# Dimitrinov74/Domain-Specific-Image-Compression

Hardware: AMD Instinct MI355X
Metric: 256x256 satellite patches encoded/s per GPU; bpp + MS-SSIM vs reference (higher is better)
Workload: dtype f32 (Winograd contractions as split-bf16 MFMA with fp32 accumulate); 1 GPU; batch=64/GPU 256x256x3 synthetic patches, modelv2 encode->decode (g_a,h_a,round,h_s,Student-t/Gaussian rate,g_s) + bpp + MS-SSIM[.3,.5,.2] on GPU + CDF tables and range coder (z,y strings) on GPU [BASELINE config 3]; global_batch=64, parallelism=per-image sharding x1, one all-reduce of 4 fp64, weights=synthetic seed 1 (checkpoints absent from the reference)

## Files before the change

### domain-specific-image-compression_amd/csrc/conv_first.hip

```cpp
#include <stdlib.h>

#include <type_traits>

#include "common.h"

namespace dsic {

typedef float floatx16 __attribute__((ext_vector_type(16)));
typedef float floatx4 __attribute__((ext_vector_type(4)));
typedef float floatx8 __attribute__((ext_vector_type(8)));
typedef __bf16 bf16x8 __attribute__((ext_vector_type(8)));

__device__ __forceinline__ void first_split8(const floatx8 v, bf16x8& hi, bf16x8& mid) {
  hi = __builtin_convertvector(v, bf16x8);
  const floatx8 back = __builtin_convertvector(hi, floatx8);
  mid = __builtin_convertvector(v - back, bf16x8);
}

template <int C, bool U8 = false, bool BF16 = false>
__global__ __launch_bounds__(256, 2) void conv_first_kernel(
    const void* __restrict__ xv, const float* __restrict__ w, const float* __restrict__ bias,
    const float* __restrict__ beta, const float* __restrict__ gamma, float* __restrict__ out, int B,
    int H, int W, int Cout, int act, int tiles_x, int tiles_y, int layout) {
  const int s2d = layout & 1, cm = layout & DSIC_LAYOUT_CM16;
  constexpr int K = 9 * C;
  constexpr int KP = (K + 1) / 2 * 2;
  constexpr int NS = KP / 2;
  constexpr int TW = 16, TH = 8, WW = TW + 2, WH = TH + 2, RS = 20;
  constexpr int EPI_STRIDE = 36;
  constexpr int WIN_FLOATS = C * WH * RS;
  constexpr int EPI_FLOATS = 4 * 32 * EPI_STRIDE;
  __shared__ __attribute__((aligned(16))) float lds[WIN_FLOATS > EPI_FLOATS ? WIN_FLOATS : EPI_FLOATS];
  constexpr int KB = (K + 15) / 16 * 16;
  constexpr int NKS = KB / 16;
  constexpr int PXB = 4 * KB + 16;
  __shared__ __attribute__((aligned(16))) unsigned char im2col[BF16 ? 128 * PXB : 16];

  const int tid = threadIdx.x, lane = tid & 63;
  const int wave = __builtin_amdgcn_readfirstlane(tid >> 6);
  const int h = lane >> 5, l31 = lane & 31;
  int bx = blockIdx.x;
  const int tile_x = bx % tiles_x;
  bx /= tiles_x;
  const int tile_y = bx % tiles_y;
  const int n = bx / tiles_y;
  const int ox0 = tile_x * TW, oy0 = tile_y * TH;

  const int col = wave * 32 + l31;
  const bool colok = col < Cout;
  float b[BF16 ? 1 : NS];
  int aoff[BF16 ? 1 : NS];
  int abase[4];
  bf16x8 bhi[BF16 ? NKS : 1], bmid[BF16 ? NKS : 1];
  if (BF16) {
#pragma unroll
    for (int ks = 0; ks < NKS; ++ks) {
      floatx8 wv;
#pragma unroll
      for (int j = 0; j < 8; ++j) {
        const int k = ks * 16 + h * 8 + j;
        wv[j] = (colok && k < K) ? w[(size_t)col * K + k] : 0.f;
      }
      first_split8(wv, bhi[ks], bmid[ks]);
    }
  } else {
#pragma unroll
    for (int s = 0; s < NS; ++s) {
      const int k = 2 * s + h;
      b[s] = (colok && k < K) ? w[(size_t)col * K + k] : 0.f;
    }
#pragma unroll
    for (int s = 0; s < NS; ++s) {
      int k = 2 * s + h;
      if (k >= K) k = 0;
      const int c = k / 9, t = k % 9;
      aoff[s] = (c * WH + t / 3) * RS + t % 3;
    }
#pragma unroll
    for (int m = 0; m < 4; ++m) {
      const int r = m * 32 + l31;
      abase[m] = (r / TW) * RS + r % TW;
    }
  }

  if (U8) {
    const unsigned char* xin = (const unsigned char*)xv + (size_t)n * C * H * W;
    for (int i = tid; i < C * WH * WW; i += 256) {
      const int c = i % C, xx = (i / C) % WW, r = i / (C * WW);
      const int gy = oy0 - 1 + r, gx = ox0 - 1 + xx;
      float v = 0.f;
      if (gy >= 0 && gy < H && gx >= 0 && gx < W) v = (float)xin[((size_t)gy * W + gx) * C + c] / 255.0f;
      lds[(c * WH + r) * RS + xx] = v;
    }
  } else {
    const float* xin = (const float*)xv + (size_t)n * C * H * W;
    for (int i = tid; i < C * WH * WW; i += 256) {
      const int c = i / (WH * WW), r = (i / WW) % WH, xx = i % WW;
      const int gy = oy0 - 1 + r, gx = ox0 - 1 + xx;
      float v = 0.f;
      if (gy >= 0 && gy < H && gx >= 0 && gx < W) v = xin[((size_t)c * H + gy) * W + gx];
      lds[(c * WH + r) * RS + xx] = v;
    }
  }
  __syncthreads();

  floatx16 acc[4];
#pragma unroll
  for (int m = 0; m < 4; ++m)
#pragma unroll
    for (int e = 0; e < 16; ++e) acc[m][e] = 0.f;
  if (BF16) {
    const int px = tid & 127, half = tid >> 7;
    const int pbase = (px / TW) * RS + px % TW;
    auto build = [&](auto half_tag) {
      constexpr int HALF = decltype(half_tag)::value;
#pragma unroll
      for (int oo = 0; oo < NKS; ++oo) {
        const int o = 2 * oo + HALF;
        floatx8 v;
#pragma unroll
        for (int j = 0; j < 8; ++j) {
          const int k = 8 * o + j;
          const int c = k / 9, t = k % 9;
          v[j] = k < K ? lds[pbase + (c * WH + t / 3) * RS + t % 3] : 0.f;
        }
        bf16x8 vh, vm;
        first_split8(v, vh, vm);
        *(bf16x8*)(im2col + px * PXB + o * 16) = vh;
        *(bf16x8*)(im2col + px * PXB + 2 * KB + o * 16) = vm;
      }
    };
    if (half == 0)
      build(std::integral_constant<int, 0>{});
    else
      build(std::integral_constant<int, 1>{});
    __syncthreads();
#pragma unroll
    for (int m = 0; m < 4; ++m) {
      const unsigned char* ap = im2col + (m * 32 + l31) * PXB + h * 16;
#pragma unroll
      for (int ks = 0; ks < NKS; ++ks) {
        const bf16x8 ah = *(const bf16x8*)(ap + ks * 32);
        const bf16x8 am = *(const bf16x8*)(ap + 2 * KB + ks * 32);
        acc[m] = __builtin_amdgcn_mfma_f32_32x32x16_bf16(ah, bmid[ks], acc[m], 0, 0, 0);
        acc[m] = __builtin_amdgcn_mfma_f32_32x32x16_bf16(am, bhi[ks], acc[m], 0, 0, 0);
        acc[m] = __builtin_amdgcn_mfma_f32_32x32x16_bf16(ah, bhi[ks], acc[m], 0, 0, 0);
      }
    }
  } else {
#pragma unroll
    for (int s = 0; s < NS; ++s) {
      float a[4];
#pragma unroll
      for (int m = 0; m < 4; ++m) a[m] = lds[abase[m] + aoff[s]];
#pragma unroll
      for (int m = 0; m < 4; ++m) acc[m] = __builtin_amdgcn_mfma_f32_32x32x2f32(a[m], b[s], acc[m], 0, 0, 0);
    }
  }
  __syncthreads();

  const float bs = colok ? bias[col] : 0.f;
  float be = 1.f, ga = 0.f;
  if (colok && act == DSIC_ACT_GDN) {
    be = beta[col];
    ga = gamma[col];
  }
  float* epi = lds + wave * (32 * EPI_STRIDE);
#pragma unroll
  for (int m = 0; m < 4; ++m) {
#pragma unroll
    for (int e = 0; e < 16; e += 2) {
      dsic_float2 v = {acc[m][e], acc[m][e + 1]};
      v = v + dsic_float2{bs, bs};
      if (act == DSIC_ACT_GDN) {
        v = gdn_pair<false>(v, dsic_float2{be, be}, dsic_float2{ga, ga});
      } else if (act == DSIC_ACT_RELU) {
        v[0] = v[0] > 0.f ? v[0] : 0.f;
        v[1] = v[1] > 0.f ? v[1] : 0.f;
      }
#pragma unroll
      for (int k = 0; k < 2; ++k) {
        const int rr = ((e + k) & 3) + 8 * ((e + k) >> 2) + 4 * h;
        epi[rr * EPI_STRIDE + l31] = v[k];
      }
    }
    __builtin_amdgcn_s_waitcnt(0xc07f);
    __builtin_amdgcn_wave_barrier();
    const int c4 = (lane & 7) * 4;
    const int nn = wave * 32 + c4;
#pragma unroll
    for (int i = 0; i < 4; ++i) {
      const int rr = (lane >> 3) + 8 * i;
      const floatx4 v = *(const floatx4*)(epi + rr * EPI_STRIDE + c4);
      const int r = m * 32 + rr;
      const int ox = ox0 + r % TW, oy = oy0 + r / TW;
      if (oy < H && ox < W && nn < Cout) {
        const int64_t pix = s2d ? (int64_t)(oy >> 1) * (W >> 1) + (ox >> 1) : (int64_t)oy * W + ox;
        const int64_t npix = s2d ? (int64_t)(H >> 1) * (W >> 1) : (int64_t)H * W;
        const int Co = s2d ? 4 * Cout : Cout, ch = s2d ? ((oy & 1) * 2 + (ox & 1)) * Cout + nn : nn;
        const size_t o = cm ? (size_t)(((int64_t)n * Co + (ch & ~15)) * npix + pix * 16 + (ch & 15))
                            : (size_t)(((int64_t)n * npix + pix) * Co + ch);
        __builtin_nontemporal_store(v, (floatx4*)(out + o));
      }
    }
    __builtin_amdgcn_s_waitcnt(0xc07f);
    __builtin_amdgcn_wave_barrier();
  }
}

__global__ void u8hwc_to_f32nchw_kernel(const unsigned char* __restrict__ in, float* __restrict__ out, int C,
                                        int HW, int64_t total) {
  const int64_t i = (int64_t)blockIdx.x * blockDim.x + threadIdx.x;
  if (i >= total) return;
  const int64_t p = i % HW;
  const int64_t bc = i / HW;
  const int c = (int)(bc % C);
  const int64_t b = bc / C;
  out[i] = (float)in[(b * HW + p) * C + c] / 255.0f;
}

}

using namespace dsic;

extern "C" int dsic_image_u8hwc_to_f32nchw(const unsigned char* x_u8_nhwc, float* out_nchw, int B, int C, int H,
                                           int W, void* stream) {
  DSIC_REQUIRE(x_u8_nhwc && out_nchw && B > 0 && C > 0 && H > 0 && W > 0, "image_u8hwc_to_f32nchw: bad argument");
  const int64_t total = (int64_t)B * C * H * W;
  hipLaunchKernelGGL(u8hwc_to_f32nchw_kernel, dim3((unsigned)((total + 255) / 256)), dim3(256), 0, (hipStream_t)stream,
                     x_u8_nhwc, out_nchw, C, H * W, total);
  return check_launch("image_u8hwc_to_f32nchw");
}

static int conv_first_launch(const void* x, bool u8, const float* w_oihw, const float* bias, const float* beta,
                             const float* gamma, float* out_nhwc, int B, int Cimg, int H, int W, int Cout, int act,
                             int s2d, void* stream) {
  DSIC_REQUIRE(x && w_oihw && bias && out_nhwc, "conv_first: null pointer");
  DSIC_REQUIRE(B > 0 && H > 0 && W > 0, "conv_first: empty tensor");
  DSIC_REQUIRE(Cimg == 3 || Cimg == 4, "conv_first: Cimg=%d must be 3 or 4", Cimg);
  DSIC_REQUIRE(Cout > 0 && Cout <= 128 && Cout % 4 == 0, "conv_first: Cout=%d must be a multiple of 4, <= 128", Cout);
  DSIC_REQUIRE(act == DSIC_ACT_NONE || act == DSIC_ACT_GDN || act == DSIC_ACT_RELU, "conv_first: act=%d", act);
  DSIC_REQUIRE(act != DSIC_ACT_GDN || (beta && gamma), "conv_first: GDN needs beta and gamma");
  DSIC_REQUIRE((s2d & ~(1 | DSIC_LAYOUT_CM16)) == 0, "conv_first: s2d=%d", s2d);
  DSIC_REQUIRE(!(s2d & 1) || (H % 2 == 0 && W % 2 == 0), "conv_first: space-to-depth output needs even H and W");
  DSIC_REQUIRE(!(s2d & DSIC_LAYOUT_CM16) || Cout % 16 == 0, "conv_first: a chunk-major output needs Cout %% 16 == 0");
  const int tx = ceil_div(W, 16), ty = ceil_div(H, 8);
  DSIC_REQUIRE((int64_t)tx * ty * B < ((int64_t)1 << 31), "conv_first: grid too large");
  dim3 grid(tx * ty * B), block(256);
  hipStream_t st = (hipStream_t)stream;
  const int use_bf16 = split_bf16();
#define DSIC_FIRST(CC, UU, BB)                                                                                        \
  hipLaunchKernelGGL((conv_first_kernel<CC, UU, BB>), grid, block, 0, st, x, w_oihw, bias, beta, gamma, out_nhwc, B, H, \
                     W, Cout, act, tx, ty, s2d)
#define DSIC_FIRST2(CC, UU) \
  do {                      \
    if (use_bf16)           \
      DSIC_FIRST(CC, UU, true); \
    else                    \
      DSIC_FIRST(CC, UU, false); \
  } while (0)
  if (Cimg == 3) {
    if (u8) DSIC_FIRST2(3, true); else DSIC_FIRST2(3, false);
  } else {
    if (u8) DSIC_FIRST2(4, true); else DSIC_FIRST2(4, false);
  }
#undef DSIC_FIRST2
#undef DSIC_FIRST
  return check_launch("conv_first");
}

extern "C" int dsic_conv_first_nchw(const float* x_nchw, const float* w_oihw, const float* bias,
                                    const float* beta, const float* gamma, float* out_nhwc, int B,
                                    int Cimg, int H, int W, int Cout, int act, int s2d, void* stream) {
  return conv_first_launch(x_nchw, false, w_oihw, bias, beta, gamma, out_nhwc, B, Cimg, H, W, Cout, act, s2d, stream);
}

extern "C" int dsic_conv_first_u8hwc(const unsigned char* x_u8_nhwc, const float* w_oihw, const float* bias,
                                     const float* beta, const float* gamma, float* out_nhwc, int B, int Cimg,
                                     int H, int W, int Cout, int act, int s2d, void* stream) {
  return conv_first_launch(x_u8_nhwc, true, w_oihw, bias, beta, gamma, out_nhwc, B, Cimg, H, W, Cout, act, s2d, stream);
}
```

### domain-specific-image-compression_amd/lib.py

```python
from __future__ import annotations

import ctypes
import os
from ctypes import c_int, c_int64, c_void_p

HERE = os.path.dirname(os.path.abspath(__file__))
LIB_PATH = os.environ.get("DSIC_LIB") or os.path.join(HERE, "libdsic_hip.so")

DSIC_OK, DSIC_EINVAL, DSIC_EHIP = 0, 1, 2
ACT_NONE, ACT_GDN, ACT_IGDN, ACT_RELU = 0, 1, 2, 3

_P = c_void_p
SIGNATURES = {
    "dsic_last_error": (ctypes.c_char_p, []),
    "dsic_abi_version": (c_int, []),
    "dsic_split_bf16": (c_int, []),
    "dsic_set_split_bf16": (c_int, [c_int]),
    "dsic_packed_conv_weight_floats": (c_int64, [c_int, c_int, c_int]),
    "dsic_pack_conv_weight": (c_int, [_P, _P, c_int, c_int, c_int, _P]),
    "dsic_pack_convT_weight": (c_int, [_P, _P, c_int, c_int, _P]),
    "dsic_convT_image_weight_floats": (c_int64, [c_int]),
    "dsic_pack_convT_image_weight": (c_int, [_P, _P, c_int, c_int, _P]),
    "dsic_image_to_nhwc8": (c_int, [_P, _P, c_int, c_int, c_int, c_int, _P]),
    "dsic_nhwc_to_nchw": (c_int, [_P, _P, c_int, c_int, c_int, c_int, _P]),
    "dsic_nchw_to_nhwc": (c_int, [_P, _P, c_int, c_int, c_int, c_int, _P]),
    "dsic_reflect_pad_br": (c_int, [_P, _P, c_int, c_int, c_int, c_int, c_int, _P]),
    "dsic_normalize_bands": (c_int, [_P, _P, _P, c_int, c_int, _P]),
    "dsic_conv2d_nhwc": (c_int, [_P, _P, _P, _P, _P, _P, c_int, c_int, c_int, c_int, c_int,
                                 c_int, c_int, c_int, _P]),
    "dsic_wino_weight_floats": (c_int64, [c_int, c_int]),
    "dsic_pack_wino_weight": (c_int, [_P, _P, c_int, c_int, _P]),
    "dsic_conv3x3_wino_nhwc": (c_int, [_P, _P, _P, _P, _P, _P, c_int, c_int, c_int, c_int, c_int, c_int, c_int, c_int,
                                       _P, _P]),
    "dsic_pack_wino_s2_weight": (c_int, [_P, _P, c_int, c_int, _P]),
    "dsic_pack_wino_convT_weight": (c_int, [_P, _P, c_int, c_int, _P]),
    "dsic_conv_transpose2d_wino_nhwc": (c_int, [_P, _P, _P, _P, _P, _P, c_int, c_int, c_int, c_int, c_int, c_int, _P,
                                                _P]),
    "dsic_wino_bf16_planes": (c_int, []),
    "dsic_wino_bf16_weight_bytes": (c_int64, [c_int, c_int]),
    "dsic_split_wino_weight_bf16": (c_int, [_P, _P, c_int, c_int, c_int, _P]),
    "dsic_conv3x3_wino_bf16_nhwc": (c_int, [_P, _P, _P, _P, _P, _P, c_int, c_int, c_int, c_int, c_int, c_int, c_int,
                                            c_int, c_int, c_int, _P, _P]),
    "dsic_wino_bf16_ksplit": (c_int, [c_int, c_int, c_int]),
    "dsic_wino_bf16_m64": (c_int, [c_int, c_int, c_int, c_int]),
    "dsic_wino_pair_chunks": (c_int, [c_int]),
    "dsic_wino_grid": (c_int, [c_int]),
    "dsic_wino_pair_schedule": (c_int, [c_int, c_int, c_int, c_int, c_int, c_int, _P, c_int]),
    "dsic_conv3x3_wino_bf16_splitk_nhwc": (c_int, [_P, _P, _P, _P, _P, _P, c_int, c_int, c_int, c_int, c_int, c_int,
                                                   c_int, c_int, c_int, c_int, c_int, _P, _P, _P]),
    "dsic_conv_transpose2d_wino_bf16_nhwc": (c_int, [_P, _P, _P, _P, _P, _P, c_int, c_int, c_int, c_int, c_int, c_int,
                                                     _P, _P]),
    "dsic_conv_transpose2d_wino_bf16_layout": (c_int, [_P, _P, _P, _P, _P, _P, c_int, c_int, c_int, c_int, c_int,
                                                       c_int, c_int, c_int, _P, _P]),
    "dsic_conv_first_nchw": (c_int, [_P, _P, _P, _P, _P, _P, c_int, c_int, c_int, c_int, c_int, c_int, c_int, _P]),
    "dsic_conv_first_u8hwc": (c_int, [_P, _P, _P, _P, _P, _P, c_int, c_int, c_int, c_int, c_int, c_int, c_int, _P]),
    "dsic_image_u8hwc_to_f32nchw": (c_int, [_P, _P, c_int, c_int, c_int, c_int, _P]),
    "dsic_conv_transpose2d_nhwc": (c_int, [_P, _P, _P, _P, _P, _P, c_int, c_int, c_int, c_int,
                                           c_int, c_int, _P]),
    "dsic_conv_transpose2d_image": (c_int, [_P, _P, _P, _P, c_int, c_int, c_int, c_int, c_int, _P]),
    "dsic_hyper_params": (c_int, [_P] * 13 + [c_int, c_int, c_int, c_int, ctypes.c_float,
                                     ctypes.c_float, _P]),
    "dsic_rate_workspace_doubles": (c_int64, [c_int]),
    "dsic_rate": (c_int, [_P] * 14 + [c_int, c_int, c_int, c_int, c_int, c_int, _P]),
    "dsic_sigma_nu_spatial": (c_int, [_P, _P, _P, _P, c_int, c_int, c_int, ctypes.c_float, ctypes.c_float, _P]),
    "dsic_student_t_bits": (c_int, [_P, _P, _P, _P, c_int64, c_int, c_int, _P]),
    "dsic_gaussian_bits": (c_int, [_P, _P, _P, c_int, c_int, c_int, _P]),
    "dsic_round": (c_int, [_P, _P, c_int64, _P]),
    "dsic_gdn_nchw": (c_int, [_P, _P, _P, _P, c_int, c_int, c_int, c_int, _P]),
    "dsic_ssim_partial_doubles": (c_int64, [c_int, c_int, c_int]),
    "dsic_ssim_level": (c_int, [_P, _P, _P, _P, c_int, c_int, c_int, ctypes.c_float, ctypes.c_float,
                                c_int, _P]),
    "dsic_ssim_level_pool_fused": (c_int, [c_int, c_int]),
    "dsic_ssim_level_pool": (c_int, [_P, _P, _P, _P, _P, _P, c_int, c_int, c_int, ctypes.c_float, ctypes.c_float,
                                     c_int, _P]),
    "dsic_avgpool2": (c_int, [_P, _P, c_int, c_int, c_int, c_int, _P]),
    "dsic_msssim_finalize": (c_int, [_P, _P, _P, c_int, c_int, c_int, c_int, _P]),
    "dsic_sqerr_per_image": (c_int, [_P, _P, _P, c_int, c_int64, c_int, _P]),
    "dsic_latent_support": (c_int, [_P, _P, _P, c_int, c_int64, c_int64, c_int, _P]),
    "dsic_cdf_tables_gauss": (c_int, [_P, _P, _P, c_int, c_int, c_int, _P, _P]),
    "dsic_cdf_tables_student": (c_int, [_P, _P, _P, _P, c_int, c_int, c_int, _P, _P]),
    "dsic_range_encode": (c_int, [_P, _P, _P, _P, _P, c_int, c_int, c_int, c_int, c_int, c_int, _P,
                                  c_int64, c_int64, _P, _P, c_int, c_int, _P]),
    "dsic_range_encode_workspace_size": (c_int64, [c_int, c_int, c_int, c_int, c_int]),
    "dsic_range_encode_ws": (c_int, [_P, _P, _P, _P, _P, c_int, c_int, c_int, c_int, c_int, c_int, _P,
                                     c_int64, c_int64, _P, _P, c_int, _P, c_int64, _P]),
    "dsic_range_encode_seg_workspace_size": (c_int64, [c_int, c_int, c_int, c_int, c_int, c_int]),
    "dsic_range_encode_seg_ws": (c_int, [_P, _P, _P, _P, _P, c_int, c_int, c_int, c_int, c_int, c_int, _P,
                                         c_int64, c_int64, _P, _P, c_int, c_int, _P, c_int64, _P]),
    "dsic_range_decode_seg": (c_int, [_P, c_int64, _P, c_int, c_int, _P, c_int, _P, c_int, _P, c_int, c_int, c_int,
                                      c_int, c_int, _P, _P, _P]),
    "dsic_container_pack_seg": (c_int, [_P, c_int64, c_int64, c_int, _P, _P, _P, c_int, ctypes.c_uint32, c_int, c_int,
                                        c_int, c_int, c_int, c_int, _P, _P, _P]),
    "dsic_tile_gather_u8": (c_int, [_P, _P, c_int, c_int, c_int, c_int, c_int, c_int, c_int, _P]),
    "dsic_tile_gather_f32": (c_int, [_P, _P, c_int, c_int, c_int, c_int, c_int, c_int, c_int, _P]),
    "dsic_tile_stitch_f32": (c_int, [_P, _P, c_int, c_int, c_int, c_int, c_int, c_int, c_int, _P]),
    "dsic_tile_stitch_u8": (c_int, [_P, _P, c_int, c_int, c_int, c_int, c_int, c_int, c_int, _P]),
    "dsic_container_pack": (c_int, [_P, c_int64, c_int64, _P, _P, _P, c_int, ctypes.c_uint32, c_int, c_int, c_int,
                                    c_int, c_int, c_int, _P, _P, _P]),
    "dsic_container_scatter": (c_int, [_P, c_int64, c_int, c_int64, _P, c_int64, _P, c_int64, _P, _P, _P, _P]),
    "dsic_strings_scatter_select": (c_int, [_P, c_int64, _P, c_int, c_int64, _P, c_int64, _P, c_int64, _P, _P]),
    "dsic_tile_stitch_window_f32": (c_int, [_P, _P, c_int, _P] + [c_int] * 9 + [_P]),
    "dsic_tile_stitch_window_u8": (c_int, [_P, _P, c_int, _P] + [c_int] * 9 + [_P]),
    "dsic_tile_gather_u8_ov": (c_int, [_P, _P] + [c_int] * 8 + [_P]),
    "dsic_tile_gather_f32_ov": (c_int, [_P, _P] + [c_int] * 8 + [_P]),
    "dsic_tile_blend_window_f32": (c_int, [_P, _P, c_int, _P] + [c_int] * 10 + [_P]),
    "dsic_tile_blend_finish_f32": (c_int, [_P, c_int, c_int, c_int, _P]),
    "dsic_tile_blend_finish_u8": (c_int, [_P, _P, c_int, c_int, c_int, _P]),
    "dsic_residual_quantize_u8": (c_int, [_P, _P, _P] + [c_int] * 5 + [_P, _P, _P]),
    "dsic_residual_tables": (c_int, [_P] + [c_int] * 6 + [_P, _P, _P, _P]),
    "dsic_residual_pack": (c_int, [_P, c_int64, c_int64, _P, _P, _P, _P] + [c_int] * 6 + [_P, _P, _P]),
    "dsic_tile_stitch_window_u8_res": (c_int, [_P, _P, c_int, _P, c_int, _P] + [c_int] * 9 + [_P]),
    "dsic_image_halve_u8": (c_int, [_P, _P, c_int, c_int, c_int, _P]),
    "dsic_image_halve_f32": (c_int, [_P, _P, c_int, c_int, c_int, _P]),
    "dsic_mask_classify_u8": (c_int, [_P] + [c_int] * 8 + [_P, _P]),
    "dsic_mask_delta_planes_u8": (c_int, [_P] + [c_int] * 6 + [_P, c_int, _P, _P, _P]),
    "dsic_mask_pack": (c_int, [_P, _P, _P, c_int, c_int, c_int, _P, _P, _P]),
    "dsic_mask_unpack": (c_int, [_P, c_int64, _P, c_int, c_int, c_int, _P, _P]),
    "dsic_mask_apply_u8": (c_int, [_P, c_int, _P, c_int, c_int, _P] + [c_int] * 9 + [_P]),
    "dsic_mask_apply_f32": (c_int, [_P, c_int, _P, c_int, c_int, _P] + [c_int] * 9 + [_P]),
    "dsic_band_range_u16": (c_int, [_P, c_int, c_int, c_int, _P, _P]),
    "dsic_tile_gather_u16": (c_int, [_P, _P] + [c_int] * 5 + [_P, c_int, c_int, _P]),
    "dsic_tile_gather_u16_ov": (c_int, [_P, _P] + [c_int] * 6 + [_P, c_int, c_int, _P]),
    "dsic_tile_stitch_window_u16": (c_int, [_P, _P, c_int, _P] + [c_int] * 9 + [_P, _P]),
    "dsic_tile_blend_finish_u16": (c_int, [_P, _P, c_int, c_int, c_int, _P, _P]),
    "dsic_image_halve_u16": (c_int, [_P, _P, c_int, c_int, c_int, _P]),
    "dsic_window_resample_u8": (c_int, [_P] + [c_int] * 10 + [_P] + [c_int] * 4 + [_P]),
    "dsic_window_resample_u16": (c_int, [_P] + [c_int] * 10 + [_P] + [c_int] * 4 + [_P]),
    "dsic_window_resample_f32": (c_int, [_P] + [c_int] * 10 + [_P] + [c_int] * 3 + [ctypes.c_float, c_int, _P]),
    "dsic_stream_create_masked":(c_int, [_P, c_int, _P]),
    "dsic_stream_destroy": (c_int, [_P]),
    "dsic_range_decode": (c_int, [_P, c_int64, _P, c_int, c_int, _P, c_int, _P, c_int, c_int, c_int,
                                  c_int, c_int, _P, _P, _P]),
    "dsic_host_normal_cdf": (ctypes.c_double, [ctypes.c_double]),
    "dsic_host_student_t_cdf": (ctypes.c_double, [ctypes.c_double, ctypes.c_double]),
    "dsic_host_gaussian_cdf_f32": (ctypes.c_float, [ctypes.c_float]),
    "dsic_host_exp_f32": (ctypes.c_float, [ctypes.c_float]),
    "dsic_host_pmf_to_uint16_cdf": (c_int, [_P, c_int, c_int, _P]),
    "dsic_host_cdf_table": (c_int, [c_int, ctypes.c_float, ctypes.c_float, c_int, c_int, _P, _P]),
}

_lib = None


def load() -> ctypes.CDLL:
    global _lib
    if _lib is None:
        if not os.path.exists(LIB_PATH):
            raise RuntimeError(
                f"{LIB_PATH} is missing: build it with "
                "`python domain-specific-image-compression_amd/build.py` "
                "(or __graft_entry__.build()); there is no CPU fallback")
        import torch
        if "GPU_MAX_HW_QUEUES" not in os.environ:
            if torch.cuda.is_initialized():
                import warnings
                warnings.warn("dsic_amd: the HIP runtime was initialised without GPU_MAX_HW_QUEUES=8; the coder's side "
                              "streams will share hardware queues with the conv stream (export it before starting python)")
            else:
                os.environ["GPU_MAX_HW_QUEUES"] = "8"
        lib = ctypes.CDLL(LIB_PATH)
        for name, (res, args) in SIGNATURES.items():
            fn = getattr(lib, name)
            fn.restype = res
            fn.argtypes = args
        _lib = lib
    return _lib


def check(status: int, what: str) -> None:
    if status == DSIC_OK:
        return
    msg = load().dsic_last_error().decode(errors="replace")
    if status == DSIC_EINVAL:
        raise ValueError(f"{what}: {msg}")
    raise RuntimeError(f"{what}: {msg}")
```

### include/dsic_hip.h

```cpp
#ifndef DSIC_HIP_H
#define DSIC_HIP_H

#include <stdint.h>

#ifdef __cplusplus
extern "C" {
#endif

#define DSIC_OK 0
#define DSIC_EINVAL 1
#define DSIC_EHIP 2

#define DSIC_ACT_NONE 0
#define DSIC_ACT_GDN 1
#define DSIC_ACT_IGDN 2
#define DSIC_ACT_RELU 3
#define DSIC_LAYOUT_CM16 2

const char* dsic_last_error(void);
int dsic_abi_version(void);

int dsic_split_bf16(void);
int dsic_set_split_bf16(int on);


int64_t dsic_packed_conv_weight_floats(int Cout, int Cin, int k);
int dsic_pack_conv_weight(const float* w_oihw, float* dst, int Cout, int Cin,
                          int k, void* stream);

int dsic_pack_convT_weight(const float* w_iohw, float* dst, int Cin, int Cout,
                           void* stream);

int64_t dsic_convT_image_weight_floats(int Cin);
int dsic_pack_convT_image_weight(const float* w_iohw, float* dst, int Cin,
                                 int Cimg, void* stream);


int dsic_image_to_nhwc8(const float* x_nchw, float* dst_nhwc8, int B, int C,
                        int H, int W, void* stream);
int dsic_nhwc_to_nchw(const float* src, float* dst, int B, int H, int W, int C,
                      void* stream);
int dsic_nchw_to_nhwc(const float* src, float* dst, int B, int C, int H, int W,
                      void* stream);

int dsic_reflect_pad_br(const float* src, float* dst, int planes, int H, int W,
                        int pad_h, int pad_w, void* stream);

int dsic_normalize_bands(const float* bands, float* out01, uint8_t* out_u8,
                         int planes, int HW, void* stream);


int dsic_conv2d_nhwc(const float* in, const float* w_packed, const float* bias,
                     const float* beta, const float* gamma, float* out, int B,
                     int H, int W, int CinP, int Cout, int k, int stride,
                     int act, void* stream);

int64_t dsic_wino_weight_floats(int Cout, int Cin);
int dsic_pack_wino_weight(const float* w_oihw, float* dst, int Cout, int Cin,
                          void* stream);
int dsic_conv3x3_wino_nhwc(const float* in, const float* u_packed,
                           const float* bias, const float* beta,
                           const float* gamma, float* out, int B, int H, int W,
                           int Cin, int Cout, int act, int s2d_out, int s2d_in,
                           void* ticket, void* stream);
int dsic_pack_wino_s2_weight(const float* w_oihw5, float* dst, int Cout, int Cs,
                             void* stream);
int dsic_pack_wino_convT_weight(const float* w_iohw5, float* dst, int Cin,
                                int Cout, void* stream);
int dsic_conv_transpose2d_wino_nhwc(const float* in, const float* u_packed4,
                                    const float* bias, const float* beta,
                                    const float* gamma, float* out, int B,
                                    int H, int W, int Cin, int Cout, int act,
                                    void* ticket, void* stream);

int dsic_wino_bf16_planes(void);
int64_t dsic_wino_bf16_weight_bytes(int Cout, int Cin);
int dsic_split_wino_weight_bf16(const float* u_f32, void* dst, int Cout, int Cin,
                                int nphase, void* stream);
int dsic_conv3x3_wino_bf16_nhwc(const float* in, const void* u_planes,
                                const float* bias, const float* beta,
                                const float* gamma, float* out, int B, int H, int W,
                                int Cin, int Cout, int act, int s2d_out, int s2d_in,
                                int out_cstride, int out_coff, void* ticket, void* stream);
int dsic_wino_bf16_ksplit(int H, int W, int Cin);
int dsic_wino_bf16_m64(int H, int W, int Cin, int nphase);
int dsic_wino_pair_chunks(int on);
int dsic_wino_grid(int n);
int dsic_wino_pair_schedule(int mode, int nchunks, int phase, int paired, int pq, int acc, int* out, int cap);
int dsic_conv3x3_wino_bf16_splitk_nhwc(const float* in, const void* u_planes,
                                       const float* bias, const float* beta,
                                       const float* gamma, float* out, int B, int H, int W,
                                       int Cin, int Cout, int act, int s2d_out, int s2d_in,
                                       int out_cstride, int out_coff, int ksplit,
                                       float* partials, void* ticket, void* stream);
int dsic_conv_transpose2d_wino_bf16_nhwc(const float* in, const void* u_planes4,
                                         const float* bias, const float* beta,
                                         const float* gamma, float* out, int B,
                                         int H, int W, int Cin, int Cout, int act,
                                         void* ticket, void* stream);
int dsic_conv_transpose2d_wino_bf16_layout(const float* in, const void* u_planes4,
                                           const float* bias, const float* beta,
                                           const float* gamma, float* out, int B,
                                           int H, int W, int Cin, int Cout, int act,
                                           int layout_in, int layout_out, void* ticket,
                                           void* stream);

int dsic_conv_first_nchw(const float* x_nchw, const float* w_oihw,
                         const float* bias, const float* beta,
                         const float* gamma, float* out_nhwc, int B, int Cimg,
                         int H, int W, int Cout, int act, int s2d_out,
                         void* stream);
int dsic_conv_first_u8hwc(const unsigned char* x_u8_nhwc, const float* w_oihw,
                          const float* bias, const float* beta, const float* gamma,
                          float* out_nhwc, int B, int Cimg, int H, int W, int Cout,
                          int act, int s2d, void* stream);
int dsic_image_u8hwc_to_f32nchw(const unsigned char* x_u8_nhwc, float* out_nchw,
                                int B, int C, int H, int W, void* stream);


int dsic_conv_transpose2d_nhwc(const float* in, const float* w_packed,
                               const float* bias, const float* beta,
                               const float* gamma, float* out, int B, int H,
                               int W, int Cin, int Cout, int act, void* stream);

int dsic_conv_transpose2d_image(const float* in, const float* w_packed,
                                const float* bias, float* out_nchw, int B,
                                int H, int W, int Cin, int Cimg, void* stream);


int dsic_hyper_params(const float* t_nhwc, const float* w1_sigma,
                      const float* b1_sigma, const float* w2_sigma,
                      const float* b2_sigma, const float* w1_nu,
                      const float* b1_nu, const float* w2_nu,
                      const float* b2_nu, float* log_sigma, float* log_nu,
                      float* sigma, float* nu, int B, int HW, int N, int M,
                      float min_nu, float max_nu, void* stream);

int64_t dsic_rate_workspace_doubles(int B);
int dsic_rate(const float* y_nhwc, const float* z_nhwc,
              const float* y_noisy_nhwc, const float* z_noisy_nhwc,
              const float* sigma, const float* nu, const float* z_log_sigma,
              float* y_hat_nhwc, float* y_tilde_nchw, float* z_tilde_nchw,
              float* nll_y_nchw, float* nll_z_nchw, double* sums, double* work,
              int B, int HWy, int M, int HWz, int N, int per_element, void* stream);

int dsic_sigma_nu_spatial(const float* log_sigma_nhwc, const float* log_nu_nhwc,
                          float* sigma_nchw, float* nu_nchw, int B, int HW, int M,
                          float min_nu, float max_nu, void* stream);

int dsic_student_t_bits(const float* x, const float* sigma, const float* nu,
                        float* out, int64_t n, int HW, int per_channel,
                        void* stream);
int dsic_gaussian_bits(const float* x, const float* log_sigma, float* out,
                       int B, int C, int HW, void* stream);

int dsic_round(const float* x, float* out, int64_t n, void* stream);

int dsic_gdn_nchw(const float* x, const float* beta, const float* gamma,
                  float* out, int B, int C, int HW, int inverse, void* stream);


int64_t dsic_ssim_partial_doubles(int planes, int H, int W);
int dsic_ssim_level(const float* X, const float* Y, double* partial,
                    double* means, int planes, int H, int W, float C1, float C2,
                    int clamp_x, void* stream);
int dsic_ssim_level_pool_fused(int H, int W);
int dsic_ssim_level_pool(const float* X, const float* Y, double* partial,
                         double* means, float* Xn, float* Yn, int planes, int H,
                         int W, float C1, float C2, int clamp_x, void* stream);
int dsic_avgpool2(const float* src, float* dst, int planes, int H, int W,
                  int clamp, void* stream);
int dsic_msssim_finalize(const double* means, const float* weights, float* out,
                         int levels, int B, int C, int relu_last, void* stream);
int dsic_sqerr_per_image(const float* a, const float* b, double* out, int B,
                         int64_t n_per_image, int clamp_a, void* stream);


int dsic_latent_support(const float* y_nchw, const float* z_nchw, int* meta,
                        int B, int64_t n_y, int64_t n_z, int tail, void* stream);

int dsic_cdf_tables_gauss(const float* sigma_z, const int* meta,
                          uint16_t* tables, int B, int N, int Lmax, int* err,
                          void* stream);
int dsic_cdf_tables_student(const float* sigma, const float* nu,
                            const int* meta, uint16_t* tables, int B, int rows,
                            int Lmax, int* err, void* stream);

int dsic_range_encode(const float* y_nchw, const float* z_nchw, const int* meta,
                      const uint16_t* tab_y, const uint16_t* tab_z, int Lmax,
                      int B, int M, int HWy, int N, int HWz, uint8_t* out,
                      int64_t cap_y, int64_t cap_z, int* lengths, int* err,
                      int streams_per_wg, int per_element_y, void* stream);

int64_t dsic_range_encode_workspace_size(int B, int M, int HWy, int N, int HWz);
int dsic_range_encode_ws(const float* y_nchw, const float* z_nchw, const int* meta,
                         const uint16_t* tab_y, const uint16_t* tab_z, int Lmax,
                         int B, int M, int HWy, int N, int HWz, uint8_t* out,
                         int64_t cap_y, int64_t cap_z, int* lengths, int* err,
                         int per_element_y, void* workspace, int64_t workspace_bytes, void* stream);

int64_t dsic_range_encode_seg_workspace_size(int B, int M, int HWy, int N, int HWz, int segs);
int dsic_range_encode_seg_ws(const float* y_nchw, const float* z_nchw, const int* meta,
                             const uint16_t* tab_y, const uint16_t* tab_z, int Lmax,
                             int B, int M, int HWy, int N, int HWz, uint8_t* out,
                             int64_t cap_seg, int64_t cap_z, int* lengths, int* err,
                             int per_element_y, int segs, void* workspace, int64_t workspace_bytes,
                             void* stream);

int dsic_range_decode(const uint8_t* in, int64_t stride, const int* lengths,
                      int lstride, int loff, const int* meta, int meta_off,
                      const uint16_t* tables, int Lmax, int B, int C, int HW,
                      int per_element, float* out_nchw, int* err, void* stream);

int dsic_range_decode_seg(const uint8_t* in, int64_t stride, const int* lengths, int lstride,
                          int loff, const int* seg_lengths, int segs, const int* meta,
                          int meta_off, const uint16_t* tables, int Lmax, int B, int C, int HW,
                          int per_element, float* out_nchw, int* err, void* stream);

int dsic_tile_gather_u8(const uint8_t* img_hwc, uint8_t* tiles, int H, int W, int C,
                        int th, int tw, int first_tile, int n_tiles, void* stream);
int dsic_tile_gather_f32(const float* img_chw, float* tiles, int H, int W, int C,
                         int th, int tw, int first_tile, int n_tiles, void* stream);
int dsic_tile_stitch_f32(const float* tiles, float* img_chw, int H, int W, int C,
                         int th, int tw, int first_tile, int n_tiles, void* stream);
int dsic_tile_stitch_u8(const float* tiles, uint8_t* img_hwc, int H, int W, int C,
                        int th, int tw, int first_tile, int n_tiles, void* stream);

int dsic_container_pack(const uint8_t* bytes, int64_t cap_z, int64_t cap_y, const int* lengths,
                        const int* meta, const int* err, int B, uint32_t tag, int My, int Hy,
                        int Wy, int Nz, int Hz, int Wz, int64_t* workspace, uint8_t* out,
                        void* stream);
int dsic_container_pack_seg(const uint8_t* bytes, int64_t cap_z, int64_t cap_seg, int segs,
                            const int* lengths, const int* meta, const int* err, int B,
                            uint32_t tag, int My, int Hy, int Wy, int Nz, int Hz, int Wz,
                            int64_t* workspace, uint8_t* out, void* stream);
int dsic_container_scatter(const uint8_t* blob, int64_t blob_bytes, int B, int64_t max_len,
                           uint8_t* zbuf, int64_t zstride, uint8_t* ybuf, int64_t ystride,
                           int* lengths, int* meta, int64_t* workspace, void* stream);

int dsic_strings_scatter_select(const uint8_t* blob, int64_t blob_bytes, const int64_t* desc,
                                int n, int64_t max_len, uint8_t* zbuf, int64_t zstride,
                                uint8_t* ybuf, int64_t ystride, int* lengths, void* stream);
int dsic_tile_stitch_window_f32(const float* tiles, const int* tile_ids, int n, float* out,
                                int H, int W, int C, int th, int tw, int wy0, int wx0, int wh,
                                int ww, void* stream);
int dsic_tile_stitch_window_u8(const float* tiles, const int* tile_ids, int n, uint8_t* out,
                               int H, int W, int C, int th, int tw, int wy0, int wx0, int wh,
                               int ww, void* stream);

int dsic_tile_gather_u8_ov(const uint8_t* img_hwc, uint8_t* tiles, int H, int W, int C, int th,
                           int tw, int overlap, int first_tile, int n_tiles, void* stream);
int dsic_tile_gather_f32_ov(const float* img_chw, float* tiles, int H, int W, int C, int th,
                            int tw, int overlap, int first_tile, int n_tiles, void* stream);
int dsic_tile_blend_window_f32(const float* tiles, const int* tile_ids, int n, float* canvas,
                               int H, int W, int C, int th, int tw, int overlap, int wy0,
                               int wx0, int wh, int ww, void* stream);
int dsic_tile_blend_finish_f32(float* canvas, int C, int h, int w, void* stream);
int dsic_tile_blend_finish_u8(const float* canvas, uint8_t* out_hwc, int C, int h, int w,
                              void* stream);

int dsic_residual_quantize_u8(const uint8_t* tiles, const float* x_hat, const int* own, int n,
                              int C, int th, int tw, int tau, float* q, int* hist, void* stream);
int dsic_residual_tables(const int* hist, int n, int C, int th, int tw, int tau, int Lmax,
                         int* meta, uint16_t* compact, uint16_t* coder, void* stream);
int dsic_residual_pack(const uint8_t* bytes, int64_t cap_z, int64_t cap_seg, const int* lengths,
                       const int* meta, const uint16_t* compact, const int* err, int n, int C,
                       int th, int tw, int tau, int Lmax, int64_t* workspace, uint8_t* out,
                       void* stream);
int dsic_tile_stitch_window_u8_res(const float* tiles, const float* q, int tau,
                                   const int* tile_ids, int n, uint8_t* out, int H, int W, int C,
                                   int th, int tw, int wy0, int wx0, int wh, int ww, void* stream);

int dsic_image_halve_u8(const uint8_t* src_hwc, uint8_t* dst_hwc, int H, int W, int C,
                        void* stream);
int dsic_image_halve_f32(const float* src_chw, float* dst_chw, int C, int H, int W,
                         void* stream);

int dsic_mask_classify_u8(const uint8_t* img_hwc, int H, int W, int C, int th, int tw, int nodata,
                          int first_tile, int n_tiles, int* counts, void* stream);
int dsic_mask_delta_planes_u8(const uint8_t* img_hwc, int H, int W, int C, int th, int tw,
                              int nodata, const int* tile_ids, int n, uint32_t* planes,
                              int* popcounts, void* stream);
int dsic_mask_pack(const uint32_t* planes, const int* popcounts, const int* tile_ids, int n,
                   int th, int tw, int64_t* workspace, uint8_t* out, void* stream);
int dsic_mask_unpack(const uint8_t* blob, int64_t blob_bytes, const int* desc, int n, int th,
                     int tw, uint32_t* planes, void* stream);
int dsic_mask_apply_u8(const uint32_t* planes, int n_planes, const int* desc, int n, int nodata,
                       uint8_t* out, int H, int W, int C, int th, int tw, int wy0, int wx0,
                       int wh, int ww, void* stream);
int dsic_mask_apply_f32(const uint32_t* planes, int n_planes, const int* desc, int n, int nodata,
                        float* out, int H, int W, int C, int th, int tw, int wy0, int wx0, int wh,
                        int ww, void* stream);

int dsic_band_range_u16(const uint16_t* img_hwc, int H, int W, int C, uint32_t* out_lohi_dev,
                        void* stream);
int dsic_tile_gather_u16(const uint16_t* img_hwc, float* tiles, int H, int W, int C, int th,
                         int tw, const uint32_t* lohi, int first_tile, int n_tiles, void* stream);
int dsic_tile_gather_u16_ov(const uint16_t* img_hwc, float* tiles, int H, int W, int C, int th,
                            int tw, int overlap, const uint32_t* lohi, int first_tile, int n_tiles,
                            void* stream);
int dsic_tile_stitch_window_u16(const float* tiles, const int* tile_ids, int n_tiles,
                                uint16_t* out, int H, int W, int C, int th, int tw, int wy0,
                                int wx0, int wh, int ww, const uint32_t* lohi, void* stream);
int dsic_tile_blend_finish_u16(const float* canvas, uint16_t* out_hwc, int C, int h, int w,
                               const uint32_t* lohi, void* stream);
int dsic_image_halve_u16(const uint16_t* src_hwc, uint16_t* dst_hwc, int H, int W, int C,
                         void* stream);

int dsic_window_resample_u8(const uint8_t* src_hwc, int sh, int sw, int sy0, int sx0, int C,
                            int shift, int y0, int x0, int h, int w, uint8_t* dst_hwc, int oh,
                            int ow, int mode, int nodata, void* stream);
int dsic_window_resample_u16(const uint16_t* src_hwc, int sh, int sw, int sy0, int sx0, int C,
                             int shift, int y0, int x0, int h, int w, uint16_t* dst_hwc, int oh,
                             int ow, int mode, int nodata, void* stream);
int dsic_window_resample_f32(const float* src_chw, int sh, int sw, int sy0, int sx0, int C,
                             int shift, int y0, int x0, int h, int w, float* dst_chw, int oh,
                             int ow, int mode, float nodata, int has_nodata, void* stream);

int dsic_stream_create_masked(const uint32_t* mask_host, int words,
                              void** stream_out);
int dsic_stream_destroy(void* stream);

double dsic_host_normal_cdf(double x);
double dsic_host_student_t_cdf(double t, double nu);
float dsic_host_gaussian_cdf_f32(float x);
float dsic_host_exp_f32(float x);
int dsic_host_pmf_to_uint16_cdf(const float* pmf_host, int L, int C,
                                uint16_t* out_host);
int dsic_host_cdf_table(int student, float sigma, float nu, int smin, int L,
                        uint16_t* out_host, uint16_t* raw_host);

#ifdef __cplusplus
}
#endif
#endif
```

Baseline: 11390 images/s.

## Make first conv persistent over tile runs with prefetched input windows

```diff
diff --git a/domain-specific-image-compression_amd/csrc/conv_first.hip b/domain-specific-image-compression_amd/csrc/conv_first.hip
--- a/domain-specific-image-compression_amd/csrc/conv_first.hip
+++ b/domain-specific-image-compression_amd/csrc/conv_first.hip
@@ -10,6 +10,7 @@
 typedef float floatx4 __attribute__((ext_vector_type(4)));
 typedef float floatx8 __attribute__((ext_vector_type(8)));
 typedef __bf16 bf16x8 __attribute__((ext_vector_type(8)));
+typedef unsigned uintx4 __attribute__((ext_vector_type(4)));
 
 __device__ __forceinline__ void first_split8(const floatx8 v, bf16x8& hi, bf16x8& mid) {
   hi = __builtin_convertvector(v, bf16x8);
@@ -17,11 +18,15 @@
   mid = __builtin_convertvector(v - back, bf16x8);
 }
 
+struct FirstTile {
+  int n, ty, tx;
+};
+
 template <int C, bool U8 = false, bool BF16 = false>
-__global__ __launch_bounds__(256, 2) void conv_first_kernel(
+__global__ __launch_bounds__(256, C == 3 ? 4 : 3) void conv_first_kernel(
     const void* __restrict__ xv, const float* __restrict__ w, const float* __restrict__ bias,
     const float* __restrict__ beta, const float* __restrict__ gamma, float* __restrict__ out, int B,
-    int H, int W, int Cout, int act, int tiles_x, int tiles_y, int layout) {
+    int H, int W, int Cout, int act, int tiles_x, int tiles_y, int layout, int run, int ntiles) {
   const int s2d = layout & 1, cm = layout & DSIC_LAYOUT_CM16;
   constexpr int K = 9 * C;
   constexpr int KP = (K + 1) / 2 * 2;
@@ -30,26 +35,29 @@
   constexpr int EPI_STRIDE = 36;
   constexpr int WIN_FLOATS = C * WH * RS;
   constexpr int EPI_FLOATS = 4 * 32 * EPI_STRIDE;
-  __shared__ __attribute__((aligned(16))) float lds[WIN_FLOATS > EPI_FLOATS ? WIN_FLOATS : EPI_FLOATS];
+  __shared__ __attribute__((aligned(16))) float lds[WIN_FLOATS];
+  __shared__ __attribute__((aligned(16))) float epi_lds[EPI_FLOATS];
   constexpr int KB = (K + 15) / 16 * 16;
   constexpr int NKS = KB / 16;
   constexpr int PXB = 4 * KB + 16;
-  __shared__ __attribute__((aligned(16))) unsigned char im2col[BF16 ? 128 * PXB : 16];
+  constexpr int OCC_PAD = 2048;
+  __shared__ __attribute__((aligned(16))) unsigned char im2col[BF16 ? 128 * PXB + OCC_PAD : 16];
+  constexpr unsigned NOWHERE = 0x80000000u;
 
   const int tid = threadIdx.x, lane = tid & 63;
   const int wave = __builtin_amdgcn_readfirstlane(tid >> 6);
   const int h = lane >> 5, l31 = lane & 31;
-  int bx = blockIdx.x;
-  const int tile_x = bx % tiles_x;
-  bx /= tiles_x;
-  const int tile_y = bx % tiles_y;
-  const int n = bx / tiles_y;
-  const int ox0 = tile_x * TW, oy0 = tile_y * TH;
+  const int t0 = blockIdx.x * run;
+  if (t0 >= ntiles) return;
+  const int cnt = ntiles - t0 < run ? ntiles - t0 : run;
+  FirstTile first;
+  first.tx = t0 % tiles_x;
+  first.ty = (t0 / tiles_x) % tiles_y;
+  first.n = (t0 / tiles_x) / tiles_y;
 
   const int col = wave * 32 + l31;
   const bool colok = col < Cout;
   float b[BF16 ? 1 : NS];
-  int aoff[BF16 ? 1 : NS];
   int abase[4];
   bf16x8 bhi[BF16 ? NKS : 1], bmid[BF16 ? NKS : 1];
   if (BF16) {
@@ -70,142 +78,191 @@
       b[s] = (colok && k < K) ? w[(size_t)col * K + k] : 0.f;
     }
 #pragma unroll
-    for (int s = 0; s < NS; ++s) {
-      int k = 2 * s + h;
-      if (k >= K) k = 0;
-      const int c = k / 9, t = k % 9;
-      aoff[s] = (c * WH + t / 3) * RS + t % 3;
-    }
-#pragma unroll
     for (int m = 0; m < 4; ++m) {
       const int r = m * 32 + l31;
       abase[m] = (r / TW) * RS + r % TW;
     }
   }
-
-  if (U8) {
-    const unsigned char* xin = (const unsigned char*)xv + (size_t)n * C * H * W;
-    for (int i = tid; i < C * WH * WW; i += 256) {
-      const int c = i % C, xx = (i / C) % WW, r = i / (C * WW);
-      const int gy = oy0 - 1 + r, gx = ox0 - 1 + xx;
-      float v = 0.f;
-      if (gy >= 0 && gy < H && gx >= 0 && gx < W) v = (float)xin[((size_t)gy * W + gx) * C + c] / 255.0f;
-      lds[(c * WH + r) * RS + xx] = v;
-    }
-  } else {
-    const float* xin = (const float*)xv + (size_t)n * C * H * W;
-    for (int i = tid; i < C * WH * WW; i += 256) {
-      const int c = i / (WH * WW), r = (i / WW) % WH, xx = i % WW;
-      const int gy = oy0 - 1 + r, gx = ox0 - 1 + xx;
-      float v = 0.f;
-      if (gy >= 0 && gy < H && gx >= 0 && gx < W) v = xin[((size_t)c * H + gy) * W + gx];
-      lds[(c * WH + r) * RS + xx] = v;
-    }
-  }
-  __syncthreads();
-
-  floatx16 acc[4];
-#pragma unroll
-  for (int m = 0; m < 4; ++m)
-#pragma unroll
-    for (int e = 0; e < 16; ++e) acc[m][e] = 0.f;
-  if (BF16) {
-    const int px = tid & 127, half = tid >> 7;
-    const int pbase = (px / TW) * RS + px % TW;
-    auto build = [&](auto half_tag) {
-      constexpr int HALF = decltype(half_tag)::value;
-#pragma unroll
-      for (int oo = 0; oo < NKS; ++oo) {
-        const int o = 2 * oo + HALF;
-        floatx8 v;
-#pragma unroll
-        for (int j = 0; j < 8; ++j) {
-          const int k = 8 * o + j;
-          const int c = k / 9, t = k % 9;
-          v[j] = k < K ? lds[pbase + (c * WH + t / 3) * RS + t % 3] : 0.f;
-        }
-        bf16x8 vh, vm;
-        first_split8(v, vh, vm);
-        *(bf16x8*)(im2col + px * PXB + o * 16) = vh;
-        *(bf16x8*)(im2col + px * PXB + 2 * KB + o * 16) = vm;
-      }
-    };
-    if (half == 0)
-      build(std::integral_constant<int, 0>{});
-    else
-      build(std::integral_constant<int, 1>{});
-    __syncthreads();
-#pragma unroll
-    for (int m = 0; m < 4; ++m) {
-      const unsigned char* ap = im2col + (m * 32 + l31) * PXB + h * 16;
-#pragma unroll
-      for (int ks = 0; ks < NKS; ++ks) {
-        const bf16x8 ah = *(const bf16x8*)(ap + ks * 32);
-        const bf16x8 am = *(const bf16x8*)(ap + 2 * KB + ks * 32);
-        acc[m] = __builtin_amdgcn_mfma_f32_32x32x16_bf16(ah, bmid[ks], acc[m], 0, 0, 0);
-        acc[m] = __builtin_amdgcn_mfma_f32_32x32x16_bf16(am, bhi[ks], acc[m], 0, 0, 0);
-        acc[m] = __builtin_amdgcn_mfma_f32_32x32x16_bf16(ah, bhi[ks], acc[m], 0, 0, 0);
-      }
-    }
-  } else {
-#pragma unroll
-    for (int s = 0; s < NS; ++s) {
-      float a[4];
-#pragma unroll
-      for (int m = 0; m < 4; ++m) a[m] = lds[abase[m] + aoff[s]];
-#pragma unroll
-      for (int m = 0; m < 4; ++m) acc[m] = __builtin_amdgcn_mfma_f32_32x32x2f32(a[m], b[s], acc[m], 0, 0, 0);
-    }
-  }
-  __syncthreads();
-
   const float bs = colok ? bias[col] : 0.f;
   float be = 1.f, ga = 0.f;
   if (colok && act == DSIC_ACT_GDN) {
     be = beta[col];
     ga = gamma[col];
   }
-  float* epi = lds + wave * (32 * EPI_STRIDE);
-#pragma unroll
-  for (int m = 0; m < 4; ++m) {
-#pragma unroll
-    for (int e = 0; e < 16; e += 2) {
-      dsic_float2 v = {acc[m][e], acc[m][e + 1]};
-      v = v + dsic_float2{bs, bs};
-      if (act == DSIC_ACT_GDN) {
-        v = gdn_pair<false>(v, dsic_float2{be, be}, dsic_float2{ga, ga});
-      } else if (act == DSIC_ACT_RELU) {
-        v[0] = v[0] > 0.f ? v[0] : 0.f;
-        v[1] = v[1] > 0.f ? v[1] : 0.f;
+
+  constexpr int NSLOT = C;
+  const bool stages = tid < WH * WW;
+  const int win_r = stages ? tid / WW - 1 : -(1 << 30), win_x = tid % WW - 1;
+  const int win_lds = stages ? (tid / WW) * RS + tid % WW : WW;
+  const int win_in = (win_r * W + win_x) * (U8 ? C : 4);
+  const int in_bytes = C * H * W * (U8 ? 1 : 4), chan_bytes = U8 ? 1 : H * W * 4;
+  auto fetch = [&](const FirstTile& t, unsigned (&raw)[NSLOT]) {
+    const int oy0 = t.ty * TH, ox0 = t.tx * TW;
+    const __amdgpu_buffer_rsrc_t rs = __builtin_amdgcn_make_buffer_rsrc(
+        (void*)((const unsigned char*)xv + (size_t)t.n * in_bytes), 0, in_bytes, 0x00020000);
+    const int org = (oy0 * W + ox0) * (U8 ? C : 4);
+    const bool in = (unsigned)(oy0 + win_r) < (unsigned)H && (unsigned)(ox0 + win_x) < (unsigned)W;
+    const unsigned off = in ? (unsigned)(org + win_in) : NOWHERE;
+#pragma unroll
+    for (int c = 0; c < C; ++c) {
+      if (U8)
+        raw[c] = __builtin_amdgcn_raw_buffer_load_b8(rs, off, c * chan_bytes, 0);
+      else
+        raw[c] = __builtin_amdgcn_raw_buffer_load_b32(rs, off, c * chan_bytes, 0);
+    }
+  };
+  auto commit = [&](const unsigned (&raw)[NSLOT]) {
+#pragma unroll
+    for (int c = 0; c < C; ++c)
+      lds[win_lds + c * (WH * RS)] = U8 ? (float)raw[c] / 255.0f : __builtin_bit_cast(float, raw[c]);
+  };
+
+  const int Ws = W >> s2d, npix = (H >> s2d) * Ws, Co = Cout << (2 * s2d);
+  const unsigned PS = cm ? 16u : (unsigned)Co;
+  auto chan = [&](int ch) { return cm ? (unsigned)(ch & ~15) * (unsigned)npix + (unsigned)(ch & 15) : (unsigned)ch; };
+  const int c4 = (lane & 7) * 4, nn = wave * 32 + c4, dx0 = lane >> 3;
+  unsigned lane_off[2];
+#pragma unroll
+  for (int j = 0; j < 2; ++j) {
+    const int dx = dx0 + 8 * j;
+    const unsigned o = s2d ? (unsigned)(dx >> 1) * PS + chan((dx & 1) * Cout + nn) : (unsigned)dx * PS + chan(nn);
+    lane_off[j] = nn < Cout ? 4u * o : NOWHERE;
+  }
+  const unsigned row_pair = 4u * (s2d ? (unsigned)Ws * PS : 2u * (unsigned)W * PS);
+  const unsigned row_odd = 4u * (s2d ? chan(2 * Cout) : (unsigned)W * PS);
+  const int out_bytes = npix * Co * 4;
+  const float* epi = epi_lds + wave * (32 * EPI_STRIDE);
+  float* epi_w = epi_lds + wave * (32 * EPI_STRIDE);
+  const int epi_rd = (lane >> 3) * EPI_STRIDE + c4;
+
+  unsigned raw[NSLOT];
+  fetch(first, raw);
+  commit(raw);
+
+  auto tiles = [&](auto act_tag) {
+    constexpr int ACT = decltype(act_tag)::value;
+    FirstTile cur = first, nxt = first;
+    for (int t = 0; t < cnt; ++t) {
+      __syncthreads();
+      const bool more = t + 1 < cnt;
+      if (more) {
+        nxt.tx = cur.tx + 1, nxt.ty = cur.ty, nxt.n = cur.n;
+        if (nxt.tx == tiles_x) nxt.tx = 0, ++nxt.ty;
+        if (nxt.ty == tiles_y) nxt.ty = 0, ++nxt.n;
+        fetch(nxt, raw);
       }
-#pragma unroll
-      for (int k = 0; k < 2; ++k) {
-        const int rr = ((e + k) & 3) + 8 * ((e + k) >> 2) + 4 * h;
-        epi[rr * EPI_STRIDE + l31] = v[k];
+
+      floatx16 acc[4];
+#pragma unroll
+      for (int m = 0; m < 4; ++m)
+#pragma unroll
+        for (int e = 0; e < 16; ++e) acc[m][e] = 0.f;
+      if (BF16) {
+        const int px = tid & 127, half = tid >> 7;
+        const int pbase = (px / TW) * RS + px % TW;
+        auto build = [&](auto half_tag) {
+          constexpr int HALF = decltype(half_tag)::value;
+#pragma unroll
+          for (int oo = 0; oo < NKS; ++oo) {
+            const int o = 2 * oo + HALF;
+            floatx8 v;
+#pragma unroll
+            for (int j = 0; j < 8; ++j) {
+              const int k = 8 * o + j;
+              const int c = k / 9, kk = k % 9;
+              v[j] = k < K ? lds[pbase + (c * WH + kk / 3) * RS + kk % 3] : 0.f;
+            }
+            bf16x8 vh, vm;
+            first_split8(v, vh, vm);
+            *(bf16x8*)(im2col + px * PXB + o * 16) = vh;
+            *(bf16x8*)(im2col + px * PXB + 2 * KB + o * 16) = vm;
+          }
+        };
+        if (half == 0)
+          build(std::integral_constant<int, 0>{});
+        else
+          build(std::integral_constant<int, 1>{});
+        __syncthreads();
+#pragma unroll
+        for (int m = 0; m < 4; ++m) {
+          const unsigned char* ap = im2col + (m * 32 + l31) * PXB + h * 16;
+#pragma unroll
+          for (int ks = 0; ks < NKS; ++ks) {
+            const bf16x8 ah = *(const bf16x8*)(ap + ks * 32);
+            const bf16x8 am = *(const bf16x8*)(ap + 2 * KB + ks * 32);
+            acc[m] = __builtin_amdgcn_mfma_f32_32x32x16_bf16(ah, bmid[ks], acc[m], 0, 0, 0);
+            acc[m] = __builtin_amdgcn_mfma_f32_32x32x16_bf16(am, bhi[ks], acc[m], 0, 0, 0);
+            acc[m] = __builtin_amdgcn_mfma_f32_32x32x16_bf16(ah, bhi[ks], acc[m], 0, 0, 0);
+          }
+        }
+      } else {
+        int hh = h;
+        asm volatile("" : "+v"(hh));
+#pragma unroll
+        for (int s = 0; s < NS; ++s) {
+          constexpr auto off = [](int k) {
+            if (k >= K) k = 0;
+            const int c = k / 9, kk = k % 9;
+            return (c * WH + kk / 3) * RS + kk % 3;
+          };
+          const int aoff = hh ? off(2 * s + 1) : off(2 * s);
+          float a[4];
+#pragma unroll
+          for (int m = 0; m < 4; ++m) a[m] = lds[abase[m] + aoff];
+#pragma unroll
+          for (int m = 0; m < 4; ++m) acc[m] = __builtin_amdgcn_mfma_f32_32x32x2f32(a[m], b[s], acc[m], 0, 0, 0);
+        }
+        __syncthreads();
       }
-    }
-    __builtin_amdgcn_s_waitcnt(0xc07f);
-    __builtin_amdgcn_wave_barrier();
-    const int c4 = (lane & 7) * 4;
-    const int nn = wave * 32 + c4;
-#pragma unroll
-    for (int i = 0; i < 4; ++i) {
-      const int rr = (lane >> 3) + 8 * i;
-      const floatx4 v = *(const floatx4*)(epi + rr * EPI_STRIDE + c4);
-      const int r = m * 32 + rr;
-      const int ox = ox0 + r % TW, oy = oy0 + r / TW;
-      if (oy < H && ox < W && nn < Cout) {
-        const int64_t pix = s2d ? (int64_t)(oy >> 1) * (W >> 1) + (ox >> 1) : (int64_t)oy * W + ox;
-        const int64_t npix = s2d ? (int64_t)(H >> 1) * (W >> 1) : (int64_t)H * W;
-        const int Co = s2d ? 4 * Cout : Cout, ch = s2d ? ((oy & 1) * 2 + (ox & 1)) * Cout + nn : nn;
-        const size_t o = cm ? (size_t)(((int64_t)n * Co + (ch & ~15)) * npix + pix * 16 + (ch & 15))
-                            : (size_t)(((int64_t)n * npix + pix) * Co + ch);
-        __builtin_nontemporal_store(v, (floatx4*)(out + o));
+
+      if (more) commit(raw);
+
+      const int oy0 = cur.ty * TH, ox0 = cur.tx * TW;
+      const __amdgpu_buffer_rsrc_t ors = __builtin_amdgcn_make_buffer_rsrc(
+          (void*)(out + (size_t)cur.n * npix * Co), 0, out_bytes, 0x00020000);
+      const unsigned tile_off = 4u * ((unsigned)((oy0 >> s2d) * Ws + (ox0 >> s2d)) * PS);
+      const unsigned col_off[2] = {ox0 + dx0 < W ? lane_off[0] : NOWHERE, ox0 + dx0 + 8 < W ? lane_off[1] : NOWHERE};
+#pragma unroll
+      for (int m = 0; m < 4; ++m) {
+#pragma unroll
+        for (int e = 0; e < 16; e += 2) {
+          dsic_float2 v = {acc[m][e], acc[m][e + 1]};
+          v = v + dsic_float2{bs, bs};
+          if (ACT == DSIC_ACT_GDN) {
+            v = gdn_pair<false>(v, dsic_float2{be, be}, dsic_float2{ga, ga});
+          } else if (ACT == DSIC_ACT_RELU) {
+            v[0] = v[0] > 0.f ? v[0] : 0.f;
+            v[1] = v[1] > 0.f ? v[1] : 0.f;
+          }
+#pragma unroll
+          for (int k = 0; k < 2; ++k) {
+            const int rr = ((e + k) & 3) + 8 * ((e + k) >> 2) + 4 * h;
+            epi_w[rr * EPI_STRIDE + l31] = v[k];
+          }
+        }
+        __builtin_amdgcn_s_waitcnt(0xc07f);
+        __builtin_amdgcn_wave_barrier();
+#pragma unroll
+        for (int i = 0; i < 4; ++i) {
+          const floatx4 v = *(const floatx4*)(epi + epi_rd + 8 * i * EPI_STRIDE);
+          const int dy = 2 * m + (i >> 1);
+          if (oy0 + dy < H)
+            __builtin_amdgcn_raw_buffer_store_b128(__builtin_bit_cast(uintx4, v), ors, col_off[i & 1],
+                                                   tile_off + (dy >> 1) * row_pair + (dy & 1) * row_odd, 2);
+        }
+        __builtin_amdgcn_s_waitcnt(0xc07f);
+        __builtin_amdgcn_wave_barrier();
       }
-    }
-    __builtin_amdgcn_s_waitcnt(0xc07f);
-    __builtin_amdgcn_wave_barrier();
-  }
+
+      cur = nxt;
+    }
+  };
+  if (act == DSIC_ACT_GDN)
+    tiles(std::integral_constant<int, DSIC_ACT_GDN>{});
+  else if (act == DSIC_ACT_RELU)
+    tiles(std::integral_constant<int, DSIC_ACT_RELU>{});
+  else
+    tiles(std::integral_constant<int, DSIC_ACT_NONE>{});
 }
 
 __global__ void u8hwc_to_f32nchw_kernel(const unsigned char* __restrict__ in, float* __restrict__ out, int C,
@@ -230,6 +287,30 @@
   hipLaunchKernelGGL(u8hwc_to_f32nchw_kernel, dim3((unsigned)((total + 255) / 256)), dim3(256), 0, (hipStream_t)stream,
                      x_u8_nhwc, out_nchw, C, H * W, total);
   return check_launch("image_u8hwc_to_f32nchw");
+}
+
+constexpr int FIRST_RUN = 2;
+static int& first_run_override() {
+  static int n = 0;
+  return n;
+}
+static int first_run(int ntiles) {
+  if (first_run_override() > 0) return first_run_override();
+  static int cus[64] = {};
+  int dev = 0;
+  if (hipGetDevice(&dev) != hipSuccess || dev < 0 || dev >= 64) dev = 0;
+  if (cus[dev] == 0 && (hipDeviceGetAttribute(&cus[dev], hipDeviceAttributeMultiprocessorCount, dev) != hipSuccess ||
+                        cus[dev] < 1))
+    cus[dev] = 256;
+  const int fill = ntiles / (8 * cus[dev]);
+  return fill >= FIRST_RUN ? FIRST_RUN : (fill < 1 ? 1 : fill);
+}
+
+extern "C" int dsic_conv_first_tiles(int n) {
+  const int was = first_run_override();
+  if (n > (1 << 16)) return -1;
+  if (n >= 0) first_run_override() = n;
+  return was;
 }
 
 static int conv_first_launch(const void* x, bool u8, const float* w_oihw, const float* bias, const float* beta,
@@ -244,14 +325,16 @@
   DSIC_REQUIRE((s2d & ~(1 | DSIC_LAYOUT_CM16)) == 0, "conv_first: s2d=%d", s2d);
   DSIC_REQUIRE(!(s2d & 1) || (H % 2 == 0 && W % 2 == 0), "conv_first: space-to-depth output needs even H and W");
   DSIC_REQUIRE(!(s2d & DSIC_LAYOUT_CM16) || Cout % 16 == 0, "conv_first: a chunk-major output needs Cout %% 16 == 0");
+  DSIC_REQUIRE((int64_t)H * W * Cout * 4 < ((int64_t)1 << 31), "conv_first: one image's output must stay below 2 GiB");
   const int tx = ceil_div(W, 16), ty = ceil_div(H, 8);
   DSIC_REQUIRE((int64_t)tx * ty * B < ((int64_t)1 << 31), "conv_first: grid too large");
-  dim3 grid(tx * ty * B), block(256);
+  const int ntiles = tx * ty * B, run = first_run(ntiles);
+  dim3 grid(ceil_div(ntiles, run)), block(256);
   hipStream_t st = (hipStream_t)stream;
   const int use_bf16 = split_bf16();
 #define DSIC_FIRST(CC, UU, BB)                                                                                        \
   hipLaunchKernelGGL((conv_first_kernel<CC, UU, BB>), grid, block, 0, st, x, w_oihw, bias, beta, gamma, out_nhwc, B, H, \
-                     W, Cout, act, tx, ty, s2d)
+                     W, Cout, act, tx, ty, s2d, run, ntiles)
 #define DSIC_FIRST2(CC, UU) \
   do {                      \
     if (use_bf16)           \
diff --git a/domain-specific-image-compression_amd/lib.py b/domain-specific-image-compression_amd/lib.py
--- a/domain-specific-image-compression_amd/lib.py
+++ b/domain-specific-image-compression_amd/lib.py
@@ -54,6 +54,7 @@
                                                        c_int, c_int, c_int, _P, _P]),
     "dsic_conv_first_nchw": (c_int, [_P, _P, _P, _P, _P, _P, c_int, c_int, c_int, c_int, c_int, c_int, c_int, _P]),
     "dsic_conv_first_u8hwc": (c_int, [_P, _P, _P, _P, _P, _P, c_int, c_int, c_int, c_int, c_int, c_int, c_int, _P]),
+    "dsic_conv_first_tiles": (c_int, [c_int]),
     "dsic_image_u8hwc_to_f32nchw": (c_int, [_P, _P, c_int, c_int, c_int, c_int, _P]),
     "dsic_conv_transpose2d_nhwc": (c_int, [_P, _P, _P, _P, _P, _P, c_int, c_int, c_int, c_int,
                                            c_int, c_int, _P]),
diff --git a/include/dsic_hip.h b/include/dsic_hip.h
--- a/include/dsic_hip.h
+++ b/include/dsic_hip.h
@@ -114,6 +114,7 @@
                           const float* bias, const float* beta, const float* gamma,
                           float* out_nhwc, int B, int Cimg, int H, int W, int Cout,
                           int act, int s2d, void* stream);
+int dsic_conv_first_tiles(int n);
 int dsic_image_u8hwc_to_f32nchw(const unsigned char* x_u8_nhwc, float* out_nchw,
                                 int B, int C, int H, int W, void* stream);
 
```

After: 11480 images/s (median of 6 runs). About the same (+0.8%).
